# sriram-0311/MC-SLAM

Measured on AMD Instinct MI355X. Metric: multi-cam frames/sec (4-cam 1280x720 @2000 kpts/cam, extract + intra-rig match), higher is better.
Workload: dtype u8; 1 GPU; 4-cam rig 1280x720, 2000 kpts/cam, extract + all-pairs intra-rig match (configs[1]); slots=4, frames_per_launch=128, cameras=4, nfeatures=2000

## Files before the change

### mc-slam_amd/csrc/mcorb_engine.cpp

```cpp
#include <stdlib.h>
#include <string.h>
#include <sys/prctl.h>
#include <time.h>

#include "mcorb_engine.h"
#include "mcorb_prof.h"

namespace mcorb {

static thread_local std::string g_err;
void set_error(const std::string &msg) { g_err = msg; }
const char *get_error() { return g_err.c_str(); }
hipError_t Rig::wait_event(hipEvent_t ev) const
{
    if (wait_mode != 2) return hipEventSynchronize(ev);
    for (int i = 0;; i++) {
        const hipError_t e = hipEventQuery(ev);
        if (e != hipErrorNotReady) return e;
        if (i < 4) { std::this_thread::yield(); continue; }
        timespec ts = {0, 20000};
        nanosleep(&ts, nullptr);
    }
}

// ... 24 lines not shown
    }
    params = p;
    ncams = ncams_; W = W_; H = H_; max_frames = max_frames_;
    max_images = ncams * max_frames;
    undist_cams.assign(ncams, UndistCam{});
    undist_set.assign(ncams, 0);
    imgud_cams.assign(ncams, UndistImageCam{});
    imgud_set.assign(ncams, 0);
    imgud_map1.assign(ncams, {});
    imgud_map2.assign(ncams, {});
    d_imgud_map1.resize(ncams);
    d_imgud_map2.resize(ncams);
    npp = ncams * (ncams - 1) / 2;
    device = p.device_id;
    HIPCHK(hipSetDevice(device));
    TRY(compute_tables(p, tab));
    std::vector<ResizeTap> taps;
    std::vector<uint16_t> lut;
    TRY(build_geometry(p, tab, W, H, geom, taps, &lut));
    for (int l = 0; l < geom.nlevels; l++)
        selp[l] = make_select_params(kMinBorder, geom.lv[l].maxBorderX, kMinBorder, geom.lv[l].maxBorderY, tab.quota[l],
                                     geom.lv[l].wCell, geom.lv[l].hCell);
    if (taps.empty()) taps.push_back(ResizeTap{0, 0, 0, 0});
    TRY(resize_windows(geom, taps, resize_win));
    TRY(d_taps.alloc(taps.size()));
    HIPCHK(hipMemcpy(d_taps, taps.data(), taps.size() * sizeof(ResizeTap), hipMemcpyHostToDevice));
    TRY(d_lut.alloc(lut.size() + 8));
    HIPCHK(hipMemcpy(d_lut, lut.data(), lut.size() * sizeof(uint16_t), hipMemcpyHostToDevice));
    {
        std::vector<uint32_t> ft;
        fast_cell_off = fast_cell_table(geom, ft);
        TRY(d_fasttab.alloc(ft.size()));
        HIPCHK(hipMemcpy(d_fasttab, ft.data(), ft.size() * sizeof(uint32_t), hipMemcpyHostToDevice));
    }
    HIPCHK(upload_umax(tab.umax));

    const int cores = usable_cores();
    const char *sync_env = getenv("MCORB_SYNC");
    wait_mode = nslots > 1 ? 2 : 0;
    if (sync_env) wait_mode = !strcmp(sync_env, "block") ? 1 : (!strcmp(sync_env, "poll") ? 2 : 0);
    const bool blocking = wait_mode == 1;
    int nthreads = p.host_threads > 0 ? p.host_threads : (wait_mode == 0 ? cores - nslots - 2 : cores - 4);
    if (p.host_threads <= 0) nthreads = std::max(2, std::min(nthreads, std::min(max_images, 16)));
    if (getenv("MCORB_HOST_THREADS")) nthreads = atoi(getenv("MCORB_HOST_THREADS"));
    nthreads = std::max(1, std::min(nthreads, 64));
    blur_planes = p.orientation != 0 || getenv("MCORB_BLUR_PLANES") != nullptr;
    copy_kernel = getenv("MCORB_COPY_KERNEL") ? atoi(getenv("MCORB_COPY_KERNEL")) != 0 : nslots == 1;
    {
        const char *e = getenv("MCORB_SELECT");
        int mode = p.selection;
        if (mode == MCORB_SELECT_AUTO && e) mode = !strcmp(e, "host") ? MCORB_SELECT_HOST : (!strcmp(e, "gpu") ? MCORB_SELECT_GPU : MCORB_SELECT_AUTO);
        if (mode != MCORB_SELECT_AUTO && mode != MCORB_SELECT_HOST && mode != MCORB_SELECT_GPU) { set_error("mcorb_params.selection: unknown mode"); return MCORB_E_ARG; }
        gpu_select = mode != MCORB_SELECT_HOST && select_fits(geom);
        if (gpu_select) HIPCHK(configure_select(geom));
        if (getenv("MCORB_SELECT_DEEP_CAP")) select_deep_cap = std::max(1, atoi(getenv("MCORB_SELECT_DEEP_CAP")));
        compact_one_copy = getenv("MCORB_COMPACT_ONE_COPY") != nullptr;
        select_prof = getenv("MCORB_SELECT_PROF") != nullptr;
        gpu_job_limit = getenv("MCORB_GPU_JOBS") ? atoi(getenv("MCORB_GPU_JOBS")) : p.gpu_jobs;
        if (gpu_job_limit < 0 || gpu_job_limit >= nslots) gpu_job_limit = 0;
        upload_pipelined = !(getenv("MCORB_UPLOAD_PIPE") && atoi(getenv("MCORB_UPLOAD_PIPE")) == 0);
        graph_every = !gpu_select ? 0 : getenv("MCORB_GRAPH") ? std::max(0, atoi(getenv("MCORB_GRAPH"))) : (nslots == 1 ? 1 : 0);
    }
    pool.reset(new WorkerPool(nthreads));
    pool_threads = nthreads;
    for (int i = 0; i < nthreads + nslots; i++) scratch.emplace_back(new SelectScratch);

    const int npairs_max = std::max(1, npp * max_frames);
    ext_cap = (int)align_up(std::max((size_t)4096, (size_t)64 * max_images), 64);
    for (int si = 0; si < nslots; si++) {
        slots.emplace_back(new Slot);
        Slot *s = slots.back().get();
        s->rig = this;
        s->index = si;
        for (Stream *st : {&s->st, &s->st_copy, &s->st_dma}) TRY(st->create(hipStreamNonBlocking));
        TRY(s->ev_x.create(hipEventDisableTiming));
        for (Event *e : {&s->ev_c, &s->ev_e, &s->ev_start, &s->ev_pyr, &s->ev_fast, &s->ev_blur, &s->ev_desc0, &s->ev_desc1, &s->ev_knn0, &s->ev_knn1, &s->ev_fin})
            TRY(e->create(hipEventDefault));
        for (Event *e : {&s->ev_tables, &s->ev_done, &s->ev_side}) TRY(e->create(blocking ? hipEventBlockingSync : hipEventDefault));
        const size_t M = (size_t)max_images;
        TRY(s->d_pyr.alloc(M * geom.imgBytes));
        HIPCHK(hipMemset(s->d_pyr, 0, M * geom.imgBytes));
        if (blur_planes) {
            TRY(s->d_blur.alloc(M * geom.imgBytes));
            HIPCHK(hipMemset(s->d_blur, 0, M * geom.imgBytes));
        }
        TRY(s->d_cellkp.alloc(M * geom.cells * geom.cellCap));
        TRY(s->d_cellcnt.alloc(M * geom.cells));
        TRY(s->d_sorted.alloc(M * geom.candCap));
        s->tbl_ints_per_image = tbl_ints(geom.bucketTotal);
        TRY(s->d_tbl.alloc(M * s->tbl_ints_per_image));
        TRY(host_alloc(s->h_tbl, M * s->tbl_ints_per_image));
        TRY(s->d_desc.alloc(M * geom.kcap * 32));
        HIPCHK(hipMemset(s->d_desc, 0, M * geom.kcap * 32));
        TRY(s->d_angles.alloc(M * geom.kcap));
        TRY(s->d_part.alloc(knn_part_entries(npairs_max, geom.kcap)));
        TRY(s->d_exp.alloc(M * geom.kcap * (size_t)kKnnExpandBytes));
        TRY(s->d_lcounts.alloc(M));
        TRY(host_alloc(s->h_cand, M * geom.hostCandCap));
        TRY(host_alloc(s->h_overflow, 16));
        TRY(s->d_knn.alloc((size_t)npairs_max * geom.kcap));
        TRY(host_alloc(s->h_mlist, (size_t)npairs_max * knn_mlist_stride(geom.kcap)));
        TRY(host_alloc(s->h_mcount, (size_t)npairs_max * knn_qblocks(geom.kcap)));
        {
            const size_t o_nsel = (size_t)ext_cap * sizeof(int);
            const size_t o_setmap = align_up(o_nsel + M * sizeof(int), 64);
            const size_t o_pairs = align_up(o_setmap + M * sizeof(int), 64);
            const size_t o_sel = align_up(o_pairs + (size_t)npairs_max * sizeof(int2), 64);
// ... 360 lines not shown
    return MCORB_OK;
}

int Rig::enqueue_back(Slot &s, const Job &j, bool then_match, bool gpu_sel)
{
    const int nimg = j.nimg;
    const bool small = s.host_results, ev_on = s.ev_on();
    if (!gpu_sel && !small) HIPCHK(hipMemcpyAsync(s.d_ctrl, s.h_ctrl, s.ctrl_bytes, hipMemcpyHostToDevice, s.st));
    if (ev_on) HIPCHK(hipEventRecord(s.ev_desc0, s.st));
    if (small && undist_on) {
        HIPCHK(hipEventRecord(s.ubuf.ev_u0, s.st));
        HIPCHK(hipStreamWaitEvent(s.st_dma, s.ubuf.ev_u0, 0));
        TRY(enqueue_undistort(s, nimg));
    }
    launch_describe(s.st, s.d_pyr, blur_planes ? s.d_blur : nullptr, geom, s.ctl.sel, s.ctl.nsel, params.orientation, s.d_desc, s.d_angles, nimg,
                    small ? s.h_desc : nullptr);
    if (ev_on) HIPCHK(hipEventRecord(s.ev_desc1, s.st));
    if (small) {
        if (then_match) TRY(enqueue_match(s, j, true));
        HIPCHK(hipGetLastError());
        if (undist_on) HIPCHK(hipStreamWaitEvent(s.st, s.ubuf.ev_u1, 0));
        if (s.bow_job) TRY(enqueue_bow(s, nimg));
        if (gpu_sel && ev_on) HIPCHK(hipEventRecord(s.ev_side, s.st));
        return MCORB_OK;
    }
    const size_t nk = (size_t)nimg * geom.kcap;
    HIPCHK(hipStreamWaitEvent(s.st_dma, s.ev_desc1, 0));
    if (!copy_kernel) HIPCHK(hipMemcpyAsync(s.h_desc, s.d_desc, nk * 32, hipMemcpyDeviceToHost, s.st_dma));
    else launch_copy_to_host(s.st_dma, s.d_desc, s.h_desc, nk * 32);
    if (gpu_sel) {
        HIPCHK(hipMemcpyAsync(s.h_ctrl + s.ctrl_nsel_off, s.d_ctrl + s.ctrl_nsel_off, s.ctrl_pairs_end - s.ctrl_nsel_off + nk * sizeof(uint32_t),
                              hipMemcpyDeviceToHost, s.st_dma));
        HIPCHK(hipMemcpyAsync(s.h_res, s.d_res, s.res_resp_off + nk, hipMemcpyDeviceToHost, s.st_dma));
    }
    if (params.orientation) HIPCHK(hipMemcpyAsync(s.h_angles, s.d_angles, nk * sizeof(float), hipMemcpyDeviceToHost, s.st_dma));
    if (undist_on) TRY(enqueue_undistort(s, nimg));
    if (s.bow_job) TRY(enqueue_bow(s, nimg));
    if (then_match) TRY(enqueue_match(s, j, true));
    HIPCHK(hipGetLastError());
    HIPCHK(hipEventRecord(s.ev_side, s.st_dma));
    return MCORB_OK;
}

int Rig::enqueue_gpu_job(Slot &s, const Job &j, bool then_match)
{
    const int nimg = j.nimg;
    (void)hipGetLastError();
    const bool small = s.host_results, ev_on = s.ev_on();
    if (then_match && !small)
        HIPCHK(hipMemcpyAsync(s.d_ctrl, s.h_ctrl, s.ctrl_pairs_end, hipMemcpyHostToDevice, s.st));
    int *d_flags = reinterpret_cast<int *>(s.d_res.get());
    if (!small) HIPCHK(hipMemsetAsync(d_flags, 0, 16 * sizeof(int), s.st));
    TRY(enqueue_front(s, nimg, s.d_tbl));
    HIPCHK(launch_select(s.st, s.d_tbl, s.d_sorted, geom, s.d_selval, s.d_selcnt, d_flags, nimg, select_deep_cap, select_prof));
    launch_assemble(s.st, s.d_selval, s.d_selcnt, geom, tab.scale, j.lap0, j.lap1, s.dc.sel, s.d_res + s.res_resp_off, s.dc.nsel,
                    reinterpret_cast<int *>(s.d_res + s.res_mono_off), d_flags, nimg, small ? s.hc.sel : nullptr,
                    small ? s.h_res + s.res_resp_off : nullptr, small ? s.h_sig : nullptr);
    if (ev_on) HIPCHK(hipEventRecord(s.ev_s, s.st));
    if (ev_on) HIPCHK(hipEventRecord(s.ev_tables, s.st));
    if (blur_planes) launch_blur(s.st, s.d_pyr, s.d_blur, geom, nimg);
    if (ev_on) HIPCHK(hipEventRecord(s.ev_blur, s.st));
    return enqueue_back(s, j, then_match, true);
}

void Rig::gpu_job_begin()
{
    if (!gpu_job_limit) return;
    std::unique_lock<std::mutex> lk(gpu_jobs_m);
    gpu_jobs_cv.wait(lk, [this] { return gpu_jobs_running < gpu_job_limit; });
    gpu_jobs_running++;
}
void Rig::gpu_job_end()
{
    if (!gpu_job_limit) return;
    {
        std::lock_guard<std::mutex> lk(gpu_jobs_m);
        gpu_jobs_running--;
    }
    gpu_jobs_cv.notify_one();
}

int Rig::run_gpu_selected(Slot &s, const Job &j, bool then_match)
{
    TRY(begin_extract(s, j));
    const int nimg = j.nimg;
    s.nimg_done = nimg;
    if (then_match) TRY(prepare_match(s, j));
    if (s.host_results)
        for (int m = 0; m < nimg; m++) static_cast<volatile unsigned long long *>(s.h_sig)[m] = 0;
    auto records = [&](int m) {
        const int n = s.hc.nsel[m];
        std::vector<mcorb_keypoint> &K = s.kps[m];
        K.resize((size_t)n);
        const uint32_t *sel = s.hc.sel + (size_t)m * geom.kcap;
        const uint8_t *rs = s.h_res + s.res_resp_off + (size_t)m * geom.kcap;
        const float *ang = params.orientation ? s.h_angles + (size_t)m * geom.kcap : nullptr;
        for (int k = 0; k < n; k++) {
            int level, x, y;
            unpack_sel(sel[k], level, x, y);
            K[k] = make_keypoint(level, x, y, (float)rs[k], ang ? ang[k] : 0.f);
        }
        s.mono[m] = reinterpret_cast<const int *>(s.h_res + s.res_mono_off)[m];
    };
    int small_flags = 0;
    auto decode_signal = [&](int m, unsigned long long w) {
        small_flags |= sel_signal_bad(w);
        const int n = std::min(sel_signal_count(w), geom.kcap);
// ... 108 lines not shown
```

### mc-slam_amd/csrc/mcorb_engine.h

```cpp
#pragma once
#include <hip/hip_runtime.h>
#include <stdint.h>

#include <algorithm>
#include <atomic>
#include <condition_variable>
#include <functional>
#include <memory>
#include <mutex>
#include <string>
#include <thread>
#include <vector>

#include "../../include/mcorb.h"
#include "mcorb_common.h"
#include "mcorb_hip.h"
#include "mcorb_kernels.h"
#include "mcorb_select.h"

namespace mcorb {

const char *get_error();

struct Tables {
// ... 220 lines not shown
    int status = MCORB_OK;
    std::string err;
    UndistBufs ubuf;
    BowBufs bbuf;
    LfBufs lbuf;
};

struct EpipolarGate {
    const double *F;
    const mcorb_keypoint *const *kps;
    const float *sigma2;
};

class Rig {
public:
    Rig() = default;
    ~Rig();
    int init(const mcorb_params &p, int ncams, int W, int H, int max_frames, int nslots);

    int upload_u8(int slot, const uint8_t *const *images, int nimg, int stride);
    int upload_staged(int slot, int nimg);
    int upload_f32(int slot, const float *const *images, int nimg, int stride_bytes, int channels);
    int submit(int slot, const Job &job);
    int run_sync(int slot, const Job &job);
    int wait(int slot);

    mcorb_params params;
    Tables tab;
    Geom geom;
    int ncams = 0, W = 0, H = 0, max_frames = 0, max_images = 0, npp = 0 ;
    int ext_cap = 0;
    int device = 0;
    DevBuf<ResizeTap> d_taps;
    DevBuf<uint16_t> d_lut;
    DevBuf<uint32_t> d_fasttab;
    int fast_cell_off = 0;
    SelectParams selp[kMaxLevels];
    int resize_win[2 * kMaxLevels] = {};
    std::vector<std::unique_ptr<Slot>> slots;
    std::unique_ptr<WorkerPool> pool;
    int pool_threads = 0;
    int gpu_job_limit = 0;
    int gpu_jobs_running = 0;
    std::mutex gpu_jobs_m;
    std::condition_variable gpu_jobs_cv;
    void gpu_job_begin();
    void gpu_job_end();
    bool upload_pipelined = true;
    std::atomic<int> graph_every{0};
    int select_deep_cap = 4096;
    bool compact_one_copy = false;
    bool select_prof = false;
    bool gpu_select = false;
    int wait_mode = 0;
    hipError_t wait_event(hipEvent_t ev) const;
    std::vector<std::unique_ptr<SelectScratch>> scratch;

    void merge_tracks(Slot &s, int f, const EpipolarGate *gate, std::vector<int32_t> &tr, int &mergeable_out) const;

    std::vector<UndistCam> undist_cams;
    std::vector<uint8_t> undist_set;
    DevBuf<UndistCam> d_undist_cams;
    bool undist_on = false;
    unsigned undist_gen = 0;
    int set_undistortion(int cam, const double *K, const double *dist, int ncoeffs);
    int undist_records(Slot &s, int m0, int n, std::vector<const mcorb_keypoint *> &out);
    int undist_default(Slot &s, int m0, int n, std::vector<const mcorb_keypoint *> &out);
    int max_pairs() const { return std::max(1, npp * max_frames); }

    std::vector<UndistImageCam> imgud_cams;
    std::vector<uint8_t> imgud_set;
    std::vector<std::vector<int16_t>> imgud_map1;
    std::vector<std::vector<uint16_t>> imgud_map2;
    std::vector<DevBuf<int16_t>> d_imgud_map1;
    std::vector<DevBuf<uint16_t>> d_imgud_map2;
    DevBuf<RemapCam> d_remap_cams;
    bool imgud_on = false;
    int set_image_undistortion(int cam, const double *K, const double *dist, int ncoeffs);
    int enqueue_remap(Slot &s, int nimg);

    struct BowBinding {
        int flags = 0, levelsup = 0, L = 0, weighting = 0, scoring = 0;
        double ratio = 0.85;
        const int *child_start = nullptr, *child_count = nullptr, *child_id = nullptr, *word_id = nullptr;
        const void *child_desc = nullptr;
        const double *weight = nullptr;
    };
    BowBinding bow_bind;
    unsigned bow_gen = 0;
    bool lf_on = false;
    int lf_total_feats = 3000;
    std::vector<mcorb_camera> lf_cams;
    DevBuf<LfCam> d_lfcams;
    unsigned lf_gen = 0;
    int set_lf(const mcorb_camera *cams, int total_feats);
    int set_vocabulary(const BowBinding &b);
    int check_job_shape(const Job &j) const;
    int lock_idle_slots(const char *who, std::vector<std::unique_lock<std::mutex>> &locks);

private:
    bool copy_kernel = false;
    bool blur_planes = false;
    void driver(Slot *s);
    int execute(Slot &s, const Job &j);
    int begin_extract(Slot &s, const Job &j);
    int enqueue_front(Slot &s, int nimg, int *tbl);
// ... 42 lines not shown
```

### mc-slam_amd/csrc/mcorb_kernels.h

```cpp
#pragma once
#include <hip/hip_runtime.h>
#include <vector>
#include "../../include/mcorb.h"
#include "mcorb_common.h"
#include "mcorb_signal.h"
#include "mcorb_undistort.h"
#include "mcorb_undistort_image.h"

namespace mcorb {

constexpr int kKnnChunk = 4096;
__host__ __device__ inline int knn_chunk_len(int npairs) { return npairs <= 12 ? 256 : npairs <= 24 ? 512 : npairs <= 48 ? 1024 : kKnnChunk; }
constexpr int kKnnQueriesPerBlock = 256;
inline int knn_qblocks(int kcap) { return (kcap + kKnnQueriesPerBlock - 1) / kKnnQueriesPerBlock; }
inline size_t knn_mlist_stride(int kcap) { return (size_t)knn_qblocks(kcap) * kKnnQueriesPerBlock; }
inline size_t knn_part_entries(int max_pairs, int kcap)
{
    size_t need = 0;
    for (int np : {12, 24, 48, max_pairs}) {
        const int n = np < max_pairs ? np : max_pairs, cl = knn_chunk_len(n);
        const size_t e = (size_t)n * ((kcap + cl - 1) / cl) * kcap;
        need = need > e ? need : e;
    }
    return need;
}
constexpr int kKnnExpandBytes = 128;

struct KnnRow { uint32_t idx, d; };
__host__ __device__ inline int knn_idx0(const KnnRow &r) { return (r.idx & 0xffffu) == 0xffffu ? -1 : (int)(r.idx & 0xffffu); }
__host__ __device__ inline int knn_idx1(const KnnRow &r) { return (r.idx >> 16) == 0xffffu ? -1 : (int)(r.idx >> 16); }
__host__ __device__ inline int knn_d0(const KnnRow &r) { return knn_idx0(r) < 0 ? -1 : (int)(r.d & 0x1ffu); }
__host__ __device__ inline int knn_d1(const KnnRow &r) { return knn_idx1(r) < 0 ? -1 : (int)((r.d >> 9) & 0x1ffu); }
__host__ __device__ inline bool knn_accept(const KnnRow &r) { return (r.d >> 18) & 1u; }

hipError_t upload_umax(const int umax[16]);
void launch_stage_f32(hipStream_t st, const float *src, int w, int h, int pitch_f, int channels, size_t img_stride_f,
                      uint8_t *pyr, const Geom &g, int nimg);
struct RemapCam { const int16_t *map1; const uint16_t *map2; int32_t mode, pad; };
__host__ __device__ inline int remap_map_pitch(int w) { return (w + 3) & ~3; }
void launch_stage_f32_raw(hipStream_t st, const float *src, int w, int h, int pitch_f, int channels, size_t img_stride_f,
                          uint8_t *raw, int nimg);
void launch_remap_u8(hipStream_t st, const uint8_t *raw, uint8_t *pyr, const Geom &g, const RemapCam *cams, int ncams, int nimg);
void launch_pyramid(hipStream_t st, uint8_t *pyr, const Geom &g, const ResizeTap *tabs, const int *win, int nimg);
int fast_cell_table(const Geom &g, std::vector<uint32_t> &tab);
void launch_fast(hipStream_t st, const uint8_t *pyr, const Geom &g, int iniTh, int minTh, const uint32_t *cellRec,
                 uint32_t *cell_kp, int *cell_cnt, int nimg);
void launch_compact(hipStream_t st, const uint32_t *cell_kp, const int *cell_cnt, const Geom &g, const uint16_t *lut,
                    uint32_t *sorted_dev, uint32_t *cand, int *tbl, int *overflow, int nimg, bool one_copy = false);
void launch_blur(hipStream_t st, const uint8_t *pyr, uint8_t *blur, const Geom &g, int nimg);
void launch_describe(hipStream_t st, const uint8_t *pyr, const uint8_t *blur, const Geom &g, const uint32_t *sel,
                     const int *nsel, int orientation, uint8_t *desc, float *angles, int nimg,
                     uint8_t *desc_host = nullptr);
void launch_knn2(hipStream_t st, const uint8_t *desc, const int *counts, const int *setmap, int nsets, const int2 *pairs, int npairs,
                 int kcap, void *expanded, int *lcounts, uint2 *part, float dist_thresh, float ratio, KnnRow *out, uint32_t *mlist,
                 int *mcount, hipEvent_t ev_exp, hipEvent_t ev_mid);

int select_cap(const Geom &g);
bool select_fits(const Geom &g);
hipError_t configure_select(const Geom &g);
hipError_t launch_select(hipStream_t st, const int *tbl, const uint32_t *sorted, const Geom &g, uint32_t *sel_val, int *sel_cnt, int *fallback, int nimg,
                         int deep_cap = 4096, bool prof = false);
void launch_assemble(hipStream_t st, const uint32_t *sel_val, const int *sel_cnt, const Geom &g, const float *scale, int lap0, int lap1,
                     uint32_t *sel, uint8_t *resp, int *nsel, int *mono, int *fallback, int nimg,
                     uint32_t *sel_h = nullptr, uint8_t *resp_h = nullptr, unsigned long long *sig_h = nullptr);
hipError_t sort_selftest(const uint64_t *in_dev, int n, uint64_t *out_dev);

void launch_undistort(hipStream_t st, const uint32_t *sel, const int *nsel, int kcap, int nimg, int ncams, const UndistCam *cams,
                      const float *scale, int nlevels, float2 *out);

void launch_copy_to_host(hipStream_t st, const void *src_dev, void *dst_host_mapped, size_t bytes);

void launch_bow_best2(hipStream_t st, const uint8_t *desc, int img0, int kcap, int ncams, int nframes, const float *yv,
                      const int *slot_of, const int2 *node_range, const int *rg_base, const int *node_feats, const int *nfeat, int4 *out);
void launch_bow_fold(hipStream_t st, const BowRes *res, const int *nsel, int kcap, int nimg, int weighting, int scoring, int *out_dev,
                     int *out_host);
void launch_bow_tables(hipStream_t st, const int *fold, int kcap, int ncams, int nframes, const int *nsel, const uint32_t *sel,
                       const float *scale, int nlevels, const float2 *undist, int *slot_of, int *node_feats, int *nfeat, int *rg_base,
                       float *yv, int2 *node_range);
void launch_bow_descend(hipStream_t st, const uint8_t *desc, int n, const int *child_start, const int *child_count,
                        const void *child_desc, const int *child_id, const int *word_id, const double *weight, int nid_level,
                        BowRes *out);

void launch_lf_tracks(hipStream_t st, const int4 *trk, const LfView *views, int ntr, const LfCam *cams, const uint8_t *desc, int kcap,
                      int ncams, LfTrackOut *out);
void launch_tri_selftest(hipStream_t st, const double *x, const double *P, const int *nv, const int *voff, int n, double *X, int *branch);

void launch_kfdb_score(hipStream_t st, const uint32_t *ids, const double *vals, const int *nbow, int stride, const uint32_t *q_ids,
                       const double *q_vals, const int *q_n, const int *q_sel, const int *q_limit, const int *e_list, int nq,
                       int max_limit, int out_stride, double *raw, int *shared);
void launch_kfdb_best2(hipStream_t st, const uint8_t *desc_a, const int *feats_a, const uint8_t *desc_b, const int *feats_b,
                       const int2 *items, int nitems, const int2 *nodes, int4 *out);
void launch_kfdb_best2_probes(hipStream_t st, const uint8_t *desc_a, const int *feats_a, const uint8_t *desc_p, size_t desc_stride,
                              const int *feats_p, size_t feats_stride, const int2 *items, int nitems, const int4 *nodes, int4 *out);
void launch_kfdb_gather(hipStream_t st, const uint8_t *desc, const int *src, int n, uint8_t *dst);

constexpr int kLmapCullT = 256;
void launch_lmap_cull(hipStream_t st, const mcorb_lmap_view *view, const double *geom, const int *cand, int n, uint32_t *masks);
void launch_lmap_put(hipStream_t st, const int *lids, int n, const double *pt, const double *normal, const uint8_t *src_desc,
                     const int *rows, double *geom, uint8_t *desc);

}
```

### mc-slam_amd/csrc/mcorb_select_gpu.hip

```cpp
#include <hip/hip_runtime.h>
#include <stdint.h>
#include <stdio.h>

#include "mcorb_common.h"
#include "mcorb_device.h"
#include "mcorb_hip.h"
#include "mcorb_kernels.h"
#include "mcorb_sortmodel.h"

namespace mcorb {

namespace {

__device__ __forceinline__ int sel_scan3(int v, int &tot)
{
    const unsigned long long b0 = __ballot(v & 1), b1 = __ballot(v & 2), b2 = __ballot(v & 4);
    tot = __popcll(b0) + 2 * __popcll(b1) + 4 * __popcll(b2);
    return lane_rank(b0) + 2 * lane_rank(b1) + 4 * lane_rank(b2) + v;
}

typedef uint4 SelNode;
constexpr int kSelDepthShift = 28;
__device__ __forceinline__ uint32_t node_code(SelNode n) { return n.x & ((1u << kSelDepthShift) - 1u); }
__device__ __forceinline__ int node_depth(SelNode n) { return (int)(n.x >> kSelDepthShift); }
__device__ __forceinline__ int node_count(SelNode n) { return (int)n.z; }

struct SelCtx {
    const int *bst;
    const uint32_t *cand;
    int D, maxDepth, H0, wCell, hCell;
    int deepCap;
    float hX;
};
struct DeepGeom { int x0, x1, y0, y1, mx0, mx1, my0, my1; };
__device__ inline DeepGeom deep_geom(const SelCtx &C, SelNode n)
{
    const int d = node_depth(n);
    const uint32_t code = node_code(n);
    const int r = (int)(code >> (2 * d));
    DeepGeom G;
    G.x0 = (int)__fmul_rn(C.hX, (float)r); G.x1 = (int)__fmul_rn(C.hX, (float)(r + 1));
    G.y0 = 0; G.y1 = C.H0;
    G.mx0 = 0; G.mx1 = 1 << 20; G.my0 = 0; G.my1 = 1 << 20;
    for (int j = 1; j <= d; j++) {
        const int q = (int)((code >> (2 * (d - j))) & 3u);
        const int sx = G.x0 + ((G.x1 - G.x0 + 1) >> 1), sy = G.y0 + ((G.y1 - G.y0 + 1) >> 1);
        if (q & 1) { G.x0 = sx; if (j > C.D) G.mx0 = sx; } else { G.x1 = sx; if (j > C.D) G.mx1 = sx; }
        if (q & 2) { G.y0 = sy; if (j > C.D) G.my0 = sy; } else { G.y1 = sy; if (j > C.D) G.my1 = sy; }
    }
    return G;
}
__device__ inline bool node_kids(const SelCtx &C, SelNode n, int cnt[4])
{
    const int d = node_depth(n);
    if (d < C.D) {
        const int sh = 2 * (C.D - d - 1);
        const int base = (int)((node_code(n) << 2) << sh);
        const int e0 = C.bst[base], e1 = C.bst[base + (1 << sh)], e2 = C.bst[base + (2 << sh)], e3 = C.bst[base + (3 << sh)], e4 = C.bst[base + (4 << sh)];
        cnt[0] = e1 - e0; cnt[1] = e2 - e1; cnt[2] = e3 - e2; cnt[3] = e4 - e3;
        return true;
// ... 14 lines not shown
}
__device__ __forceinline__ SelNode node_child(SelNode n, int q, int cnt)
{
    const int x0 = (int)(n.y & 0xffffu), x1 = (int)(n.y >> 16);
    const int sx = x0 + ((x1 - x0 + 1) >> 1);
    const int cx0 = (q & 1) ? sx : x0, cx1 = (q & 1) ? x1 : sx;
    return SelNode{((node_code(n) << 2) | (uint32_t)q) | ((uint32_t)(node_depth(n) + 1) << kSelDepthShift), (uint32_t)cx0 | ((uint32_t)cx1 << 16), (uint32_t)cnt, 0u};
}
__device__ inline uint32_t node_best(const SelCtx &C, const uint2 *win, SelNode n)
{
    const int d = node_depth(n);
    if (d <= C.D) {
        const int sh = 2 * (C.D - d);
        const int b0 = (int)(node_code(n) << sh), nb = 1 << sh;
        uint32_t bestKey = 0, bestVal = 0;
        for (int b = 0; b < nb; b++) {
            const uint2 w = win[b0 + b];
            if (w.x > bestKey) { bestKey = w.x; bestVal = w.y; }
        }
        return bestVal;
    }
    const int b = (int)(node_code(n) >> (2 * (d - C.D)));
    const DeepGeom G = deep_geom(C, n);
    uint32_t best = 0;
    int bestR = -1;
    unsigned long long bestO = 0;
    for (int k = C.bst[b]; k < C.bst[b + 1]; k++) {
        const uint32_t c = C.cand[k];
        const int x = cand_x(c), y = cand_y(c), r = cand_resp(c);
        if (!(x >= G.mx0 && x < G.mx1 && y >= G.my0 && y < G.my1) || r < bestR) continue;
        const unsigned long long o = (((((unsigned long long)((y - 3) / C.hCell) << 12) | (unsigned long long)((x - 3) / C.wCell)) << 12 | (unsigned long long)y) << 12) |
                                     (unsigned long long)x;
        if (r > bestR || o < bestO) { bestR = r; best = c; bestO = o; }
    }
    return best;
}
__device__ __forceinline__ uint32_t kids_info(const int cnt[4])
{
    uint32_t m = 0x100u;
#pragma unroll
    for (int q = 0; q < 4; q++) m |= (cnt[q] > 0 ? 1u << q : 0u) | (cnt[q] > 1 ? 16u << q : 0u);
    return m;
}

struct SelLds {
    int *bst;
    const uint2 *win;
    SelNode *list[2];
    uint64_t *exp[2];
    uint16_t *ta, *tb;
    uint32_t *blk;
    int *stk;
};
constexpr int kSelStack = 3 * 48;
__host__ __device__ inline size_t sel_lds_bytes(int B, int cap) { return (size_t)(B + 1 + 3) / 4 * 16 + (size_t)(B + 1) / 2 * 16 + (size_t)cap * (2 * 16 + 2 * 8 + 2 * 2 + 4) + kSelStack * 4; }

__device__ void wave_std_sort(uint64_t *a, int n, uint64_t *out, SelLds &S)
{
    const int lane = lane_id();
    uint16_t *lp = S.ta, *rp = S.tb;
    if (n <= 0) return;
    int sp = 0;
    if (lane == 0) { S.stk[0] = 0; S.stk[1] = n; S.stk[2] = 2 * sm_lg(n); }
    sp = 1;
    wave_lds_sync();
    while (sp > 0) {
        sp--;
        int f = wave_uniform(S.stk[3 * sp]), l = wave_uniform(S.stk[3 * sp + 1]), dl = wave_uniform(S.stk[3 * sp + 2]);
        while (l - f > 16) {
            if (dl == 0) {
                if (lane == 0) sm_heap_sort(a, f, l);
                wave_lds_sync();
                break;
            }
            dl--;
            const int mid = f + (l - f) / 2;
            const uint32_t ka = sm_key(a[f + 1]), kb = sm_key(a[mid]), kc = sm_key(a[l - 1]);
            const int mi = sm_median3(ka, kb, kc, f + 1, mid, l - 1);
            if (lane == 0) { const uint64_t t = a[f]; a[f] = a[mi]; a[mi] = t; }
            wave_lds_sync();
            const uint32_t p = mi == f + 1 ? ka : (mi == mid ? kb : kc);
            if (l - f - 1 <= 64) {
                const int i = f + 1 + lane;
                const bool in = i < l;
                const uint32_t k = sm_key(a[min(i, l - 1)]);
                const bool isL = in && !(k < p), isR = in && !(p < k);
                const unsigned long long bl = __ballot(isL), br = __ballot(isR);
                const int nL = __popcll(bl), nR = __popcll(br);
                const int below = lane_rank(bl);
                const int above = __popcll(lane == 63 ? 0ull : br >> (lane + 1));
                const int Lj = __builtin_amdgcn_ds_permute((isL ? below : nL + (lane - below)) << 2, i);
                const int Rj = __builtin_amdgcn_ds_permute((isR ? above : nR + (63 - lane - above)) << 2, i);
                const bool ok = lane < min(nL, nR) && Lj < Rj;
                const int s = __popcll(__ballot(ok));
                const int nextL = s < nL ? __builtin_amdgcn_readlane(Lj, s) : (1 << 30), lastR = s > 0 ? __builtin_amdgcn_readlane(Rj, s - 1) : (1 << 30);
                const int cut = min(nextL, lastR);
                if (lane < s) {
                    const uint64_t ex = a[Lj], ey = a[Rj];
                    a[Lj] = ey; a[Rj] = ex;
                }
                if (lane == 0) { S.stk[3 * sp] = cut; S.stk[3 * sp + 1] = l; S.stk[3 * sp + 2] = dl; }
                sp++;
                l = cut;
                wave_lds_sync();
                continue;
            }
            int nL = 0, nR = 0;
            for (int c0 = f + 1; c0 < l; c0 += 64) {
// ... 148 lines not shown
        const int t = t0 + lane;
        const uint32_t inf = t < k ? einfo[t] : 0u;
        if (inf & 0x200u) badk = 1;
        int tot;
        (void)sel_scan3(__popc(inf & 15u), tot);
        Hc += tot;
    }
    if (__ballot(badk != 0) != 0ull || Hc + n - k > cap) { fb = 1; mOut = 0; return n; }
    int crun = 0, erun = 0;
    for (int t0 = 0; t0 < k; t0 += 64) {
        const int t = t0 + lane;
        const uint32_t inf = t < k ? einfo[t] : 0u;
        const uint32_t mask = inf & 15u, emask = (inf >> 4) & 15u;
        const int nc = __popc(mask), ne = __popc(emask);
        int ctot, etot;
        const int cin = sel_scan3(nc, ctot), ein = sel_scan3(ne, etot);
        if (t < k) {
            const uint32_t pos0 = (uint32_t)srt[m - 1 - t];
            const SelNode nd = in[pos0];
            divided[pos0] = 1;
            int cnt[4];
            (void)node_kids(C, nd, cnt);
            const int cincl = crun + cin, eexcl = erun + ein - ne;
#pragma unroll
            for (int q = 0; q < 4; q++) {
                if (!((mask >> q) & 1u)) continue;
                const SelNode ch = node_child(nd, q, cnt[q]);
                const int pos = Hc - cincl + __popc(mask >> (q + 1));
                out[pos] = ch;
                if ((emask >> q) & 1u)
                    exp[eexcl + __popc(emask & ((1u << q) - 1u))] = ((uint64_t)(((uint32_t)cnt[q] << 12) | (ch.y & 0xffffu)) << 32) | (uint32_t)pos;
            }
        }
        crun += ctot;
        erun += etot;
    }
    wave_lds_sync();
    int trun = 0;
    for (int c0 = 0; c0 < n; c0 += 64) {
        const int i = c0 + lane;
        const bool keep = i < n && divided[i] == 0;
        const unsigned long long b = __ballot(keep);
        if (keep) out[Hc + lane_rank(b, trun)] = in[i];
        trun += __popcll(b);
    }
    wave_lds_sync();
    mOut = erun;
    return Hc + trun;
}

}

__global__ __launch_bounds__(64) void k_select(const int *__restrict__ tbl, const uint32_t *__restrict__ sorted, Geom g, uint32_t *__restrict__ out_val, int *__restrict__ out_cnt,
                                               int selcap, int ldsB, int ldsCap, int deepCap, int *__restrict__ fallback, unsigned long long *__restrict__ prof)
{
    extern __shared__ __attribute__((aligned(16))) uint8_t sel_sh[];
    const int lane = lane_id();
    const int img = blockIdx.x, level = blockIdx.y;
    int prof_i = 0;
    auto stamp = [&]() {
        if (prof && img == 0 && lane == 0 && prof_i < 32) prof[level * 32 + prof_i++] = __builtin_amdgcn_s_memtime();
    };
    stamp();
    const LevelGeom &L = g.lv[level];
    const int N = L.quota, D = L.depth, B = L.nBuckets, cap = ldsCap;
    const int *tb = tbl + (size_t)img * tbl_ints(g.bucketTotal);
    const int ncand = tb[kTblLvlOff + level + 1] - tb[kTblLvlOff + level];
    int *ocnt = out_cnt + (size_t)img * g.nlevels + level;
    uint32_t *oval = out_val + ((size_t)img * g.nlevels + level) * selcap;
    if (ncand <= 0) {
        if (lane == 0) *ocnt = 0;
        return;
    }
    SelLds S;
    {
        uint8_t *p = sel_sh;
        S.bst = reinterpret_cast<int *>(p); p += (size_t)(ldsB + 1 + 3) / 4 * 16;
        S.win = reinterpret_cast<const uint2 *>(p); p += (size_t)(ldsB + 1) / 2 * 16;
        S.list[0] = reinterpret_cast<SelNode *>(p); p += (size_t)cap * 16;
        S.list[1] = reinterpret_cast<SelNode *>(p); p += (size_t)cap * 16;
        S.exp[0] = reinterpret_cast<uint64_t *>(p); p += (size_t)cap * 8;
        S.exp[1] = reinterpret_cast<uint64_t *>(p); p += (size_t)cap * 8;
        S.blk = reinterpret_cast<uint32_t *>(p); p += (size_t)cap * 4;
        S.ta = reinterpret_cast<uint16_t *>(p); p += (size_t)cap * 2;
        S.tb = reinterpret_cast<uint16_t *>(p); p += (size_t)cap * 2;
        S.stk = reinterpret_cast<int *>(p);
    }
    SelCtx C;
    C.bst = S.bst;
    C.cand = sorted + (size_t)img * g.candCap + tb[kTblLvlOff + level];
    C.D = D;
    {
        int rootBits = 0;
        while ((1 << rootBits) < L.nIni) rootBits++;
        C.maxDepth = min(14, (kSelDepthShift - rootBits) / 2);
    }
    C.H0 = L.maxBorderY - kMinBorder;
    C.wCell = L.wCell > 0 ? L.wCell : (1 << 20);
    C.hCell = L.hCell > 0 ? L.hCell : (1 << 20);
    C.hX = L.hX;
    C.deepCap = deepCap;
    {
        const int *bsrc = tb + kTblHead + L.bucket0;
        const uint2 *wsrc = reinterpret_cast<const uint2 *>(tb + tbl_win_off(g.bucketTotal)) + L.bucket0;
        uint2 *wdst = const_cast<uint2 *>(S.win);
        for (int b = lane; b <= B; b += 64) S.bst[b] = bsrc[b];
        for (int b = lane; b < B; b += 64) wdst[b] = wsrc[b];
    }
    wave_lds_sync();
    stamp();
    int n, m = 0, fb = 0, cur = 0;
    {
        const int i = lane;
        bool keep = false;
        SelNode nd{0, 0, 0, 0};
        if (i < L.nIni) {
            nd.x = (uint32_t)i;
            nd.y = (uint32_t)(int)__fmul_rn(L.hX, (float)i) | ((uint32_t)(int)__fmul_rn(L.hX, (float)(i + 1)) << 16);
            nd.z = (uint32_t)(S.bst[(i + 1) << (2 * D)] - S.bst[i << (2 * D)]);
            keep = nd.z > 0;
        }
        const unsigned long long b = __ballot(keep);
        if (keep) S.list[0][lane_rank(b)] = nd;
        n = __popcll(b);
    }
    wave_lds_sync();
    if (L.nIni > 64 || L.nIni < 1 || N + 8 > cap || C.maxDepth < D) fb = 1;
    bool finish = fb != 0;
    while (!finish) {
        const int prev = n;
        n = full_pass(S, C, S.list[cur], n, S.list[cur ^ 1], S.exp[0], cap, m, fb);
        stamp();
        if (fb) break;
        cur ^= 1;
        if (n >= N || n == prev) break;
        if (n + 3 * m > N) {
            int ecur = 0;
            while (true) {
                const int prev2 = n;
                wave_std_sort(S.exp[ecur], m, S.exp[ecur ^ 1], S);
                stamp();
                int m2 = 0;
                n = careful_round(S, C, S.list[cur], n, S.list[cur ^ 1], S.exp[ecur ^ 1], m, S.exp[ecur], N, cap, m2, fb);
                stamp();
                if (fb) break;
                cur ^= 1;
                m = m2;
                if (n >= N || n == prev2) break;
            }
            break;
        }
    }
    if (fb || n > selcap) {
        if (lane == 0) { *ocnt = -1; atomicOr(fallback, 1); }
        return;
    }
    const SelNode *list = S.list[cur];
    for (int i = lane; i < n; i += 64) oval[i] = node_best(C, S.win, list[i]);
    if (lane == 0) *ocnt = n;
    stamp();
}

struct AssembleParams { float scale[kMaxLevels]; int lap0, lap1; };
__global__ __launch_bounds__(64 * kMaxLevels) void k_assemble(const uint32_t *__restrict__ sel_val, const int *__restrict__ sel_cnt, Geom g, AssembleParams P,
                                                               int selcap, uint32_t *__restrict__ sel, uint8_t *__restrict__ resp, int *__restrict__ nsel,
                                                               int *__restrict__ mono, int *__restrict__ fallback, uint32_t *__restrict__ sel_h,
                                                               uint8_t *__restrict__ resp_h, unsigned long long *sig_h)
{
    __shared__ int s_cnt[kMaxLevels], s_st[kMaxLevels];
    __shared__ uint32_t s_chk[kMaxLevels];
    const int lane = lane_id(), level = threadIdx.x >> 6, img = blockIdx.x;
    const int c = sel_cnt[(size_t)img * g.nlevels + level];
    const uint32_t *v = sel_val + ((size_t)img * g.nlevels + level) * selcap;
    const float sc = P.scale[level], lo = (float)P.lap0, hi = (float)P.lap1;
    auto is_stereo = [&](uint32_t cd) {
        float kx = (float)(cand_x(cd) + kMinBorder);
        if (level != 0) kx = __fmul_rn(kx, sc);
        return kx >= lo && kx <= hi;
    };
    constexpr int kAsmRegs = 8;
// ... 29 lines not shown
            if (sig_h) __hip_atomic_exchange(&sig_h[img], sel_signal(bad, 0, 0, 0), __ATOMIC_RELEASE, __HIP_MEMORY_SCOPE_SYSTEM);
        }
        return;
    }
    uint32_t *so = sel + (size_t)img * g.kcap;
    uint8_t *ro = resp + (size_t)img * g.kcap;
    int monoIndex = monoBefore, stereoIndex = total - 1 - stereoBefore;
    uint32_t chk = 0;
    auto place = [&](int i, uint32_t cd) {
        const bool valid = i < c;
        const bool stereo = valid && is_stereo(cd);
        const unsigned long long bs = __ballot(stereo), bm = __ballot(valid && !stereo);
        if (valid) {
            const int pos = stereo ? stereoIndex - lane_rank(bs) : monoIndex + lane_rank(bm);
            const uint32_t ps = pack_sel(level, cand_x(cd) + kMinBorder, cand_y(cd) + kMinBorder);
            so[pos] = ps;
            ro[pos] = (uint8_t)cand_resp(cd);
            if (sel_h) {
                sel_h[(size_t)img * g.kcap + pos] = ps;
                resp_h[(size_t)img * g.kcap + pos] = (uint8_t)cand_resp(cd);
                chk ^= sel_check(ps, (uint8_t)cand_resp(cd), pos);
            }
        }
        stereoIndex -= __popcll(bs);
        monoIndex += __popcll(bm);
    };
#pragma unroll
    for (int u = 0; u < kAsmRegs; u++)
        if (u * 64 < c) place(u * 64 + lane, vr[u]);
    for (int c0 = 64 * kAsmRegs; c0 < c; c0 += 64) place(c0 + lane, c0 + lane < c ? v[c0 + lane] : 0u);
    if (threadIdx.x == 0) { nsel[img] = total; mono[img] = monoAll; }
    if (sig_h) {
#pragma unroll
        for (int o = 32; o >= 1; o >>= 1) chk ^= __shfl_xor(chk, o);
        if (lane == 0) s_chk[level] = chk;
        __threadfence_system();
        __syncthreads();
        if (threadIdx.x == 0) {
            uint32_t x = 0;
            for (int l = 0; l < g.nlevels; l++) x ^= s_chk[l];
            __hip_atomic_exchange(&sig_h[img], sel_signal(0, total, monoAll, x), __ATOMIC_RELEASE, __HIP_MEMORY_SCOPE_SYSTEM);
        }
    }
}


int select_cap(const Geom &g)
{
    int q = 1;
    for (int l = 0; l < g.nlevels; l++) q = q > g.lv[l].quota ? q : g.lv[l].quota;
    return (q + 64 + 63) & ~63;
}

constexpr size_t kSelLdsMax = 160 * 1024;
static size_t select_lds(const Geom &g, int &B)
{
    B = 1;
    for (int l = 0; l < g.nlevels; l++) B = B > g.lv[l].nBuckets ? B : g.lv[l].nBuckets;
    return sel_lds_bytes(B, select_cap(g));
}

bool select_fits(const Geom &g)
{
    int B;
    for (int l = 0; l < g.nlevels; l++)
        if (g.lv[l].nIni > 64) return false;
    return select_cap(g) <= 65535 && select_lds(g, B) <= kSelLdsMax;
}

hipError_t configure_select(const Geom &g)
{
    int B;
    if (select_lds(g, B) <= 64 * 1024) return hipSuccess;
    return hipFuncSetAttribute((const void *)k_select, hipFuncAttributeMaxDynamicSharedMemorySize, (int)kSelLdsMax);
}

hipError_t launch_select(hipStream_t st, const int *tbl, const uint32_t *sorted, const Geom &g, uint32_t *sel_val, int *sel_cnt, int *fallback, int nimg, int deep_cap, bool prof_on)
{
    int B;
    const int cap = select_cap(g);
    const size_t lds = select_lds(g, B);
    if (!select_fits(g)) return hipErrorInvalidValue;
    static HostBuf<unsigned long long> prof;
    if (prof_on && !prof) (void)prof.alloc(kMaxLevels * 32, hipHostMallocMapped);
    if (prof_on && prof) {
        static int calls = 0;
        if (++calls == 40) {
            (void)hipStreamSynchronize(st);
            for (int l = 0; l < g.nlevels; l++) {
                fprintf(stderr, "[select prof] level %d:", l);
                for (int i = 1; i < 32 && prof[l * 32 + i]; i++) fprintf(stderr, " %llu", prof[l * 32 + i] - prof[l * 32 + i - 1]);
                fprintf(stderr, "\n");
            }
        }
        for (int i = 0; i < kMaxLevels * 32; i++) prof[i] = 0;
    }
    hipLaunchKernelGGL(k_select, dim3(nimg, g.nlevels), dim3(64), lds, st, tbl, sorted, g, sel_val, sel_cnt, cap, B, cap, deep_cap, fallback, prof_on ? prof : nullptr);
    return hipGetLastError();
}

void launch_assemble(hipStream_t st, const uint32_t *sel_val, const int *sel_cnt, const Geom &g, const float *scale, int lap0, int lap1,
                     uint32_t *sel, uint8_t *resp, int *nsel, int *mono, int *fallback, int nimg, uint32_t *sel_h, uint8_t *resp_h,
                     unsigned long long *sig_h)
{
    AssembleParams P;
    for (int l = 0; l < kMaxLevels; l++) P.scale[l] = l < g.nlevels ? scale[l] : 1.f;
    P.lap0 = lap0; P.lap1 = lap1;
    hipLaunchKernelGGL(k_assemble, dim3(nimg), dim3(64 * g.nlevels), 0, st, sel_val, sel_cnt, g, P, select_cap(g), sel, resp, nsel, mono, fallback, sel_h, resp_h, sig_h);
}

__global__ __launch_bounds__(64) void k_sort_selftest(const uint64_t *__restrict__ in, int n, uint64_t *__restrict__ out, int cap)
{
    extern __shared__ __attribute__((aligned(16))) uint8_t sel_sh[];
    SelLds S;
    uint8_t *p = sel_sh;
    S.bst = reinterpret_cast<int *>(p); p += 16;
    S.list[0] = S.list[1] = nullptr;
    S.exp[0] = reinterpret_cast<uint64_t *>(p); p += (size_t)cap * 8;
    S.exp[1] = reinterpret_cast<uint64_t *>(p); p += (size_t)cap * 8;
    S.blk = reinterpret_cast<uint32_t *>(p); p += (size_t)cap * 4;
    S.ta = reinterpret_cast<uint16_t *>(p); p += (size_t)cap * 2;
    S.tb = reinterpret_cast<uint16_t *>(p); p += (size_t)cap * 2;
    S.stk = reinterpret_cast<int *>(p);
    for (int i = lane_id(); i < n; i += 64) S.exp[0][i] = in[i];
    wave_lds_sync();
    wave_std_sort(S.exp[0], n, S.exp[1], S);
    for (int i = lane_id(); i < n; i += 64) out[i] = S.exp[1][i];
}

hipError_t sort_selftest(const uint64_t *in_dev, int n, uint64_t *out_dev)
{
    const int cap = (n + 63) & ~63;
    const size_t lds = 16 + (size_t)cap * (8 + 8 + 4 + 2 + 2) + kSelStack * 4;
    if (n < 0 || cap > 6000 || lds > 160 * 1024) return hipErrorInvalidValue;
    if (lds > 64 * 1024) {
        const hipError_t e = hipFuncSetAttribute((const void *)k_sort_selftest, hipFuncAttributeMaxDynamicSharedMemorySize, (int)lds);
        if (e != hipSuccess) return e;
    }
    hipLaunchKernelGGL(k_sort_selftest, dim3(1), dim3(64), lds, 0, in_dev, n, out_dev, cap);
    return hipDeviceSynchronize();
}

}
```

Measured before the change: 40340 frames/s.

## Size select-kernel LDS per pyramid level and launch levels in occupancy classes

Replaces the single select launch, which reserved LDS for the largest level's bucket count and quota, with per-level LDS carving. Levels are sorted by LDS footprint and grouped into up to three launch classes by a simple cost model using CU count and waves-per-CU. Small levels can then run with less LDS and higher occupancy. The cost is extra kernel launches and a heuristic class split that may not match real timing.

```diff
diff --git a/mc-slam_amd/csrc/mcorb_engine.cpp b/mc-slam_amd/csrc/mcorb_engine.cpp
--- a/mc-slam_amd/csrc/mcorb_engine.cpp
+++ b/mc-slam_amd/csrc/mcorb_engine.cpp
@@ -100,7 +100,7 @@
         if (mode == MCORB_SELECT_AUTO && e) mode = !strcmp(e, "host") ? MCORB_SELECT_HOST : (!strcmp(e, "gpu") ? MCORB_SELECT_GPU : MCORB_SELECT_AUTO);
         if (mode != MCORB_SELECT_AUTO && mode != MCORB_SELECT_HOST && mode != MCORB_SELECT_GPU) { set_error("mcorb_params.selection: unknown mode"); return MCORB_E_ARG; }
         gpu_select = mode != MCORB_SELECT_HOST && select_fits(geom);
-        if (gpu_select) HIPCHK(configure_select(geom));
+        if (gpu_select) HIPCHK(configure_select(geom, sel_plan));
         if (getenv("MCORB_SELECT_DEEP_CAP")) select_deep_cap = std::max(1, atoi(getenv("MCORB_SELECT_DEEP_CAP")));
         compact_one_copy = getenv("MCORB_COMPACT_ONE_COPY") != nullptr;
         select_prof = getenv("MCORB_SELECT_PROF") != nullptr;
@@ -567,7 +567,7 @@
     int *d_flags = reinterpret_cast<int *>(s.d_res.get());
     if (!small) HIPCHK(hipMemsetAsync(d_flags, 0, 16 * sizeof(int), s.st));
     TRY(enqueue_front(s, nimg, s.d_tbl));
-    HIPCHK(launch_select(s.st, s.d_tbl, s.d_sorted, geom, s.d_selval, s.d_selcnt, d_flags, nimg, select_deep_cap, select_prof));
+    HIPCHK(launch_select(s.st, s.d_tbl, s.d_sorted, geom, sel_plan, s.d_selval, s.d_selcnt, d_flags, nimg, select_deep_cap, select_prof));
     launch_assemble(s.st, s.d_selval, s.d_selcnt, geom, tab.scale, j.lap0, j.lap1, s.dc.sel, s.d_res + s.res_resp_off, s.dc.nsel,
                     reinterpret_cast<int *>(s.d_res + s.res_mono_off), d_flags, nimg, small ? s.hc.sel : nullptr,
                     small ? s.h_res + s.res_resp_off : nullptr, small ? s.h_sig : nullptr);
diff --git a/mc-slam_amd/csrc/mcorb_engine.h b/mc-slam_amd/csrc/mcorb_engine.h
--- a/mc-slam_amd/csrc/mcorb_engine.h
+++ b/mc-slam_amd/csrc/mcorb_engine.h
@@ -296,6 +296,7 @@
     bool compact_one_copy = false;
     bool select_prof = false;
     bool gpu_select = false;
+    SelPlan sel_plan{};
     int wait_mode = 0;
     hipError_t wait_event(hipEvent_t ev) const;
     std::vector<std::unique_ptr<SelectScratch>> scratch;
diff --git a/mc-slam_amd/csrc/mcorb_kernels.h b/mc-slam_amd/csrc/mcorb_kernels.h
--- a/mc-slam_amd/csrc/mcorb_kernels.h
+++ b/mc-slam_amd/csrc/mcorb_kernels.h
@@ -3,6 +3,7 @@
 #include <vector>
 #include "../../include/mcorb.h"
 #include "mcorb_common.h"
+#include "mcorb_select_levels.h"
 #include "mcorb_signal.h"
 #include "mcorb_undistort.h"
 #include "mcorb_undistort_image.h"
@@ -57,9 +58,9 @@
 
 int select_cap(const Geom &g);
 bool select_fits(const Geom &g);
-hipError_t configure_select(const Geom &g);
-hipError_t launch_select(hipStream_t st, const int *tbl, const uint32_t *sorted, const Geom &g, uint32_t *sel_val, int *sel_cnt, int *fallback, int nimg,
-                         int deep_cap = 4096, bool prof = false);
+hipError_t configure_select(const Geom &g, SelPlan &plan);
+hipError_t launch_select(hipStream_t st, const int *tbl, const uint32_t *sorted, const Geom &g, const SelPlan &plan, uint32_t *sel_val, int *sel_cnt, int *fallback,
+                         int nimg, int deep_cap = 4096, bool prof = false);
 void launch_assemble(hipStream_t st, const uint32_t *sel_val, const int *sel_cnt, const Geom &g, const float *scale, int lap0, int lap1,
                      uint32_t *sel, uint8_t *resp, int *nsel, int *mono, int *fallback, int nimg,
                      uint32_t *sel_h = nullptr, uint8_t *resp_h = nullptr, unsigned long long *sig_h = nullptr);
diff --git a/mc-slam_amd/csrc/mcorb_select_gpu.hip b/mc-slam_amd/csrc/mcorb_select_gpu.hip
--- a/mc-slam_amd/csrc/mcorb_select_gpu.hip
+++ b/mc-slam_amd/csrc/mcorb_select_gpu.hip
@@ -6,6 +6,7 @@
 #include "mcorb_device.h"
 #include "mcorb_hip.h"
 #include "mcorb_kernels.h"
+#include "mcorb_select_levels.h"
 #include "mcorb_sortmodel.h"
 
 namespace mcorb {
@@ -126,8 +127,6 @@
     uint32_t *blk;
     int *stk;
 };
-constexpr int kSelStack = 3 * 48;
-__host__ __device__ inline size_t sel_lds_bytes(int B, int cap) { return (size_t)(B + 1 + 3) / 4 * 16 + (size_t)(B + 1) / 2 * 16 + (size_t)cap * (2 * 16 + 2 * 8 + 2 * 2 + 4) + kSelStack * 4; }
 
 __device__ void wave_std_sort(uint64_t *a, int n, uint64_t *out, SelLds &S)
 {
@@ -382,18 +381,18 @@
 }
 
 __global__ __launch_bounds__(64) void k_select(const int *__restrict__ tbl, const uint32_t *__restrict__ sorted, Geom g, uint32_t *__restrict__ out_val, int *__restrict__ out_cnt,
-                                               int selcap, int ldsB, int ldsCap, int deepCap, int *__restrict__ fallback, unsigned long long *__restrict__ prof)
+                                               int selcap, SelLevels lv, SelClassLevels cls, int deepCap, int *__restrict__ fallback, unsigned long long *__restrict__ prof)
 {
     extern __shared__ __attribute__((aligned(16))) uint8_t sel_sh[];
     const int lane = lane_id();
-    const int img = blockIdx.x, level = blockIdx.y;
+    const int img = blockIdx.x, level = cls.level[blockIdx.y];
     int prof_i = 0;
     auto stamp = [&]() {
         if (prof && img == 0 && lane == 0 && prof_i < 32) prof[level * 32 + prof_i++] = __builtin_amdgcn_s_memtime();
     };
     stamp();
     const LevelGeom &L = g.lv[level];
-    const int N = L.quota, D = L.depth, B = L.nBuckets, cap = ldsCap;
+    const int N = L.quota, D = L.depth, B = L.nBuckets, cap = lv.cap[level];
     const int *tb = tbl + (size_t)img * tbl_ints(g.bucketTotal);
     const int ncand = tb[kTblLvlOff + level + 1] - tb[kTblLvlOff + level];
     int *ocnt = out_cnt + (size_t)img * g.nlevels + level;
@@ -404,17 +403,17 @@
     }
     SelLds S;
     {
-        uint8_t *p = sel_sh;
-        S.bst = reinterpret_cast<int *>(p); p += (size_t)(ldsB + 1 + 3) / 4 * 16;
-        S.win = reinterpret_cast<const uint2 *>(p); p += (size_t)(ldsB + 1) / 2 * 16;
-        S.list[0] = reinterpret_cast<SelNode *>(p); p += (size_t)cap * 16;
-        S.list[1] = reinterpret_cast<SelNode *>(p); p += (size_t)cap * 16;
-        S.exp[0] = reinterpret_cast<uint64_t *>(p); p += (size_t)cap * 8;
-        S.exp[1] = reinterpret_cast<uint64_t *>(p); p += (size_t)cap * 8;
-        S.blk = reinterpret_cast<uint32_t *>(p); p += (size_t)cap * 4;
-        S.ta = reinterpret_cast<uint16_t *>(p); p += (size_t)cap * 2;
-        S.tb = reinterpret_cast<uint16_t *>(p); p += (size_t)cap * 2;
-        S.stk = reinterpret_cast<int *>(p);
+        const SelCarve c = sel_carve(lv.B[level], cap);
+        S.bst = reinterpret_cast<int *>(sel_sh + c.bst);
+        S.win = reinterpret_cast<const uint2 *>(sel_sh + c.win);
+        S.list[0] = reinterpret_cast<SelNode *>(sel_sh + c.list[0]);
+        S.list[1] = reinterpret_cast<SelNode *>(sel_sh + c.list[1]);
+        S.exp[0] = reinterpret_cast<uint64_t *>(sel_sh + c.exp[0]);
+        S.exp[1] = reinterpret_cast<uint64_t *>(sel_sh + c.exp[1]);
+        S.blk = reinterpret_cast<uint32_t *>(sel_sh + c.blk);
+        S.ta = reinterpret_cast<uint16_t *>(sel_sh + c.ta);
+        S.tb = reinterpret_cast<uint16_t *>(sel_sh + c.tb);
+        S.stk = reinterpret_cast<int *>(sel_sh + c.stk);
     }
     SelCtx C;
     C.bst = S.bst;
@@ -455,7 +454,7 @@
         n = __popcll(b);
     }
     wave_lds_sync();
-    if (L.nIni > 64 || L.nIni < 1 || N + 8 > cap || C.maxDepth < D) fb = 1;
+    if (L.nIni > 64 || L.nIni < 1 || N + 8 > cap || 4 * L.nIni > cap || B > lv.B[level] || C.maxDepth < D) fb = 1;
     bool finish = fb != 0;
     while (!finish) {
         const int prev = n;
@@ -591,35 +590,30 @@
     return (q + 64 + 63) & ~63;
 }
 
-constexpr size_t kSelLdsMax = 160 * 1024;
-static size_t select_lds(const Geom &g, int &B)
-{
-    B = 1;
-    for (int l = 0; l < g.nlevels; l++) B = B > g.lv[l].nBuckets ? B : g.lv[l].nBuckets;
-    return sel_lds_bytes(B, select_cap(g));
-}
-
 bool select_fits(const Geom &g)
 {
-    int B;
     for (int l = 0; l < g.nlevels; l++)
-        if (g.lv[l].nIni > 64) return false;
-    return select_cap(g) <= 65535 && select_lds(g, B) <= kSelLdsMax;
-}
-
-hipError_t configure_select(const Geom &g)
-{
-    int B;
-    if (select_lds(g, B) <= 64 * 1024) return hipSuccess;
+        if (g.lv[l].nIni > 64 || sel_lds_bytes(g.lv[l].nBuckets, select_level_cap(g.lv[l].quota)) > kSelLdsMax) return false;
+    return select_cap(g) <= 65535;
+}
+
+hipError_t configure_select(const Geom &g, SelPlan &plan)
+{
+    int dev = 0, ncu = 0;
+    hipError_t e = hipGetDevice(&dev);
+    if (e == hipSuccess) e = hipDeviceGetAttribute(&ncu, hipDeviceAttributeMultiprocessorCount, dev);
+    if (e != hipSuccess) return e;
+    plan = select_plan(g, ncu);
+    if (g.nlevels < 1 || plan.bytes[plan.order[0]] <= 64 * 1024) return hipSuccess;
     return hipFuncSetAttribute((const void *)k_select, hipFuncAttributeMaxDynamicSharedMemorySize, (int)kSelLdsMax);
 }
 
-hipError_t launch_select(hipStream_t st, const int *tbl, const uint32_t *sorted, const Geom &g, uint32_t *sel_val, int *sel_cnt, int *fallback, int nimg, int deep_cap, bool prof_on)
-{
-    int B;
+hipError_t launch_select(hipStream_t st, const int *tbl, const uint32_t *sorted, const Geom &g, const SelPlan &plan, uint32_t *sel_val, int *sel_cnt, int *fallback, int nimg,
+                         int deep_cap, bool prof_on)
+{
     const int cap = select_cap(g);
-    const size_t lds = select_lds(g, B);
-    if (!select_fits(g)) return hipErrorInvalidValue;
+    if (!select_fits(g) || plan.ncu < 1 || nimg < 1) return hipErrorInvalidValue;
+    const SelClasses classes = select_classes(plan, g, nimg);
     static HostBuf<unsigned long long> prof;
     if (prof_on && !prof) (void)prof.alloc(kMaxLevels * 32, hipHostMallocMapped);
     if (prof_on && prof) {
@@ -631,10 +625,22 @@
                 for (int i = 1; i < 32 && prof[l * 32 + i]; i++) fprintf(stderr, " %llu", prof[l * 32 + i] - prof[l * 32 + i - 1]);
                 fprintf(stderr, "\n");
             }
+            for (int c = 0; c < classes.nclasses; c++) {
+                const SelClass &K = classes.cls[c];
+                int wg = 0;
+                (void)hipOccupancyMaxActiveBlocksPerMultiprocessor(&wg, (const void *)k_select, 64, K.bytes);
+                fprintf(stderr, "[select prof] class %d: %u bytes of LDS, %d waves per CU, levels", c, K.bytes, wg);
+                for (int i = 0; i < K.nlev; i++) fprintf(stderr, " %d (%u)", K.lv.level[i], plan.bytes[K.lv.level[i]]);
+                fprintf(stderr, "\n");
+            }
         }
         for (int i = 0; i < kMaxLevels * 32; i++) prof[i] = 0;
     }
-    hipLaunchKernelGGL(k_select, dim3(nimg, g.nlevels), dim3(64), lds, st, tbl, sorted, g, sel_val, sel_cnt, cap, B, cap, deep_cap, fallback, prof_on ? prof : nullptr);
+    for (int c = 0; c < classes.nclasses; c++) {
+        const SelClass &K = classes.cls[c];
+        hipLaunchKernelGGL(k_select, dim3(nimg, K.nlev), dim3(64), K.bytes, st, tbl, sorted, g, sel_val, sel_cnt, cap, plan.lv, K.lv, deep_cap, fallback,
+                           prof_on ? prof : nullptr);
+    }
     return hipGetLastError();
 }
 
diff --git a/mc-slam_amd/csrc/mcorb_select_levels.h b/mc-slam_amd/csrc/mcorb_select_levels.h
--- /dev/null
+++ b/mc-slam_amd/csrc/mcorb_select_levels.h
@@ -0,0 +1,109 @@
+#pragma once
+#include <stddef.h>
+#include <stdint.h>
+
+#include "mcorb_common.h"
+
+namespace mcorb {
+
+constexpr int kSelStack = 3 * 48;
+constexpr size_t kSelLdsMax = 160 * 1024;
+constexpr size_t kSelLdsGranule = 1280;
+constexpr int kSelMaxWaves = 32;
+constexpr int kSelMaxClasses = 3;
+
+struct SelCarve { uint32_t bst, win, list[2], exp[2], blk, ta, tb, stk, end; };
+__host__ __device__ inline SelCarve sel_carve(int B, int cap)
+{
+    SelCarve c;
+    uint32_t p = 0;
+    c.bst = p; p += (uint32_t)(B + 1 + 3) / 4 * 16;
+    c.win = p; p += (uint32_t)(B + 1) / 2 * 16;
+    c.list[0] = p; p += (uint32_t)cap * 16;
+    c.list[1] = p; p += (uint32_t)cap * 16;
+    c.exp[0] = p; p += (uint32_t)cap * 8;
+    c.exp[1] = p; p += (uint32_t)cap * 8;
+    c.blk = p; p += (uint32_t)cap * 4;
+    c.ta = p; p += (uint32_t)cap * 2;
+    c.tb = p; p += (uint32_t)cap * 2;
+    c.stk = p; p += (uint32_t)kSelStack * 4;
+    c.end = p;
+    return c;
+}
+__host__ __device__ inline size_t sel_lds_bytes(int B, int cap) { return sel_carve(B, cap).end; }
+
+inline int select_level_cap(int quota) { return ((quota > 1 ? quota : 1) + 64 + 63) & ~63; }
+
+struct SelLevels { int B[kMaxLevels], cap[kMaxLevels]; };
+struct SelClassLevels { int level[kMaxLevels]; };
+struct SelClass { int nlev; SelClassLevels lv; uint32_t bytes; };
+struct SelClasses { int nclasses; SelClass cls[kSelMaxClasses]; };
+struct SelPlan {
+    SelLevels lv;
+    uint32_t bytes[kMaxLevels];
+    int order[kMaxLevels];
+    int ncu;
+};
+
+inline int sel_waves_per_cu(size_t bytes)
+{
+    const size_t alloc = (bytes + kSelLdsGranule - 1) / kSelLdsGranule * kSelLdsGranule;
+    const size_t w = alloc ? kSelLdsMax / alloc : (size_t)kSelMaxWaves;
+    return (int)(w < (size_t)kSelMaxWaves ? w : (size_t)kSelMaxWaves);
+}
+
+inline SelPlan select_plan(const Geom &g, int ncu)
+{
+    SelPlan P{};
+    P.ncu = ncu > 0 ? ncu : 1;
+    const int n = g.nlevels;
+    for (int l = 0; l < n; l++) {
+        P.lv.B[l] = g.lv[l].nBuckets;
+        P.lv.cap[l] = select_level_cap(g.lv[l].quota);
+        P.bytes[l] = (uint32_t)sel_lds_bytes(P.lv.B[l], P.lv.cap[l]);
+        P.order[l] = l;
+    }
+    for (int i = 1; i < n; i++)
+        for (int j = i; j > 0 && P.bytes[P.order[j]] > P.bytes[P.order[j - 1]]; j--) { const int t = P.order[j]; P.order[j] = P.order[j - 1]; P.order[j - 1] = t; }
+    return P;
+}
+
+constexpr double kSelBoundary = 30.0;
+inline SelClasses select_classes(const SelPlan &P, const Geom &g, int nimg)
+{
+    const int n = g.nlevels;
+    const int *order = P.order;
+    auto run_cost = [&](int a, int b) {
+        if (a >= b) return 0.0;
+        double sum = 0, longest = 0;
+        for (int i = a; i < b; i++) {
+            const double q = (double)(g.lv[order[i]].quota > 1 ? g.lv[order[i]].quota : 1);
+            sum += q;
+            longest = longest > q ? longest : q;
+        }
+        const double work = sum * (double)nimg / ((double)P.ncu * (double)sel_waves_per_cu(P.bytes[order[a]]));
+        return (work > longest ? work : longest) + kSelBoundary;
+    };
+    int best1 = n, best2 = n;
+    double best = run_cost(0, n);
+    for (int pass = 0; pass < 2; pass++)
+        for (int c1 = 1; c1 < n; c1++)
+            for (int c2 = pass ? c1 + 1 : n; c2 < (pass ? n : n + 1); c2++) {
+                const double c = run_cost(0, c1) + run_cost(c1, c2) + run_cost(c2, n);
+                if (c < best * (1.0 - 1e-9)) { best = c; best1 = c1; best2 = c2; }
+            }
+    SelClasses R{};
+    const int cut[kSelMaxClasses + 1] = {0, best1, best2, n};
+    for (int k = 0; k < kSelMaxClasses; k++) {
+        if (cut[k] >= cut[k + 1]) continue;
+        SelClass &C = R.cls[R.nclasses++];
+        C.bytes = P.bytes[order[cut[k]]];
+        bool used[kMaxLevels] = {};
+        for (int i = cut[k]; i < cut[k + 1]; i++) used[order[i]] = true;
+        for (int l = 0; l < n; l++)
+            if (used[l]) C.lv.level[C.nlev++] = l;
+    }
+    return R;
+}
+
+}
```

New measurement: 40420 frames/s (median of 5 runs). No clear change (+0.2%).
